# Chris10M/Ev2Hands

Measured on AMD Instinct MI355X. Metric: event-windows/sec at B=256 N=2048 (f16x2), higher is better.
Workload: dtype f32 (each f32 operand split into 2 fp16 planes with per-window power-of-two range scaling, 3 plane products per MAC on the f16 MFMA, f32 accumulate); 1 GPU; TEHNet.forward+MANO both hands, B=256/GPU N=2048 C=4 fp32, E-clouds, random-init 342-key checkpoint, synthetic MANO-shaped assets; global_batch=256, points=2048, channels=4, precision=f16x2, forwards_in_flight=1, world_size_seen=1, parallelism=batch-shard x1

## Files before the change

ev2hands_amd/_lib.py:

```python
from __future__ import annotations

import ctypes as C
import os

_HERE = os.path.dirname(os.path.abspath(__file__))
LIB_PATH = os.environ.get("EV2H_LIB_PATH") or os.path.join(_HERE, "libev2hands_hip.so")

vp = C.c_void_p
ci = C.c_int


class GemmDesc(C.Structure):
    _fields_ = [("X", vp), ("ldx", ci), ("W", vp), ("ldw", ci), ("Y", vp), ("ldy", ci),
                ("M", ci), ("N", ci), ("K", ci),
                ("bias", vp), ("bias_group_rows", ci), ("ldbias", ci), ("relu", ci),
                ("post_scale", vp), ("post_shift", vp),
                ("taps", ci), ("rows_per_seq", ci), ("rowmax_rows", ci), ("precision", ci), ("Ws", vp), ("ws_tile_rows", ci), ("w_unscale", C.c_float),
                ("x_amax", vp), ("x_amax2", vp), ("x_group_rows", ci), ("y_amax", vp), ("y_group_rows", ci), ("y_scale", vp),
                ("y_bound_w", C.c_float), ("y_bound_b", C.c_float), ("skinny", ci)]


class SaDesc(C.Structure):
    _fields_ = [("P1", vp), ("ldp", ci), ("pts4", vp), ("ctr4", vp), ("gidx", vp),
                ("W1x", vp), ("W2", vp), ("b2", vp), ("W3", vp), ("b3", vp),
# ... 45 lines not shown
    _fields_ = [("name", C.c_char_p), ("data", vp), ("dtype", ci), ("ndim", ci), ("shape", C.c_int64 * 4)]


DT_F32, DT_F64, DT_I64 = 0, 1, 2
LOSS_INTER_SHAPE, LOSS_INTER_TRANSL, LOSS_INTER_J3D, LOSS_HAND, LOSS_PER_HAND = 0, 1, 2, 3, 9
LOSS_H_GLOBAL_ORIENT, LOSS_H_HAND_POSE, LOSS_H_SHAPE, LOSS_H_RJ3D, LOSS_H_J3D, LOSS_H_TRANSL, LOSS_H_REG_BETAS, LOSS_H_REG_POSE, LOSS_H_J2D = range(9)
LOSS_NT = LOSS_HAND + 2 * LOSS_PER_HAND
LOSS_NSTATE = LOSS_NT + 6
PACK_EQUALIZE, PACK_HOST_ONLY, PACK_UNEQUALIZED_OK = 1, 2, 4
FAM_SA, FAM_ROWS, FAM_QCONV, FAM_DENSE, FAM_ALL = 1, 2, 4, 8, 15


def pack_f16_families(mask: int) -> int:
    return (int(mask) & 15) << 8
W_EQUALIZED, W_UNEQUALIZED_OK = 1, 2
ABI_VERSION = 8

PREC = {"f32": 0, "bf16": 1, "f16x2": 2, "bf16x3": 3, "f16": 4}


class ManoConsts(C.Structure):
    _fields_ = [("hands_mean", vp), ("comps", vp), ("blend_T", vp), ("v_template", vp),
                ("J_template", vp), ("J_shape", vp), ("weights", vp),
                ("tips", C.c_int32 * 5), ("ncomps", C.c_int32)]


class Outputs(C.Structure):
    _fields_ = [("class_logits", vp), ("params", vp * 2), ("vertices", vp * 2), ("joints", vp * 2),
                ("logits_stride", C.c_size_t), ("params_stride", C.c_size_t), ("vertices_stride", C.c_size_t), ("joints_stride", C.c_size_t)]


EXPORTS = [
    "ev2h_abi_version", "ev2h_source_hash", "ev2h_build_defs", "ev2h_last_error", "ev2h_init", "ev2h_set_side_stream", "ev2h_side_stream_probe", "ev2h_streams_concurrent", "ev2h_bind_stream", "ev2h_shader_clock_probe", "ev2h_struct_sizes",
    "ev2h_prep_points", "ev2h_fps", "ev2h_fps_multi", "ev2h_ball_query", "ev2h_three_nn_interp",
    "ev2h_gemm", "ev2h_transpose_logits", "ev2h_sa_mlp_max", "ev2h_fp_mlp", "ev2h_tile_geometry",
    "ev2h_attn_sim", "ev2h_attn_sim_folded", "ev2h_attn_sim_folded_scratch", "ev2h_attn_context", "ev2h_mano", "ev2h_mano_rotations",
    "ev2h_workspace_bytes", "ev2h_forward", "ev2h_workspace_buffer", "ev2h_workspace_buffer_ex", "ev2h_profile_set", "ev2h_range_report_entries", "ev2h_range_report",
    "ev2h_pack_weights", "ev2h_packed_free", "ev2h_packed_weights", "ev2h_packed_bytes", "ev2h_packed_tensor_count", "ev2h_packed_tensor",
    "ev2h_packed_equalization_count", "ev2h_packed_equalization", "ev2h_packed_weight_spread_count", "ev2h_packed_weight_spread", "ev2h_pack_sa_image_bytes", "ev2h_pack_sa_images",
    "ev2h_pack_gemm_image_bytes", "ev2h_pack_gemm_image", "ev2h_plane_unscale",
    "ev2h_event_window_build", "ev2h_event_window_timesort", "ev2h_event_window_sample", "ev2h_joint_metrics", "ev2h_mesh_collisions", "ev2h_mesh_collisions_ws", "ev2h_mesh_collisions_scratch_bytes", "ev2h_collision_penalty",
    "ev2h_event_window_pixels", "ev2h_demo_point_panels", "ev2h_render_scratch_bytes", "ev2h_render_hands",
    "ev2h_event_stream_links", "ev2h_event_stream_ends", "ev2h_event_stream_walk", "ev2h_event_window_build_ranges",
    "ev2h_event_window_sample_seeded", "ev2h_fps_init_seeded", "ev2h_joint_metrics_frames", "ev2h_eval_accumulate",
    "ev2h_events_undistort",
    "ev2h_event_window_build_s_ranges", "ev2h_joint_metrics_f32_frames", "ev2h_segmentation_score", "ev2h_eval_s_accumulate",
    "ev2h_loss_terms", "ev2h_loss_accumulate",
    "ev2h_event_window_build_s_ranges_aug",
    "ev2h_event_window_build_ranges_flip", "ev2h_finetune_resolve", "ev2h_finetune_targets",
]

_lib = None


class Ev2hError(RuntimeError):
    pass


def lib() -> C.CDLL:
    global _lib
    if _lib is not None:
        return _lib
    import torch
    if not os.path.exists(LIB_PATH):
        raise Ev2hError(f"{LIB_PATH} is missing: build the HIP library first "
                        f"(python -m ev2hands_amd.build). There is no CPU fallback.")
    L = C.CDLL(LIB_PATH)
    if not os.environ.get("EV2H_LIB_PATH"):
        from . import build as _build
        try:
            L.ev2h_source_hash.restype = C.c_char_p
            have = L.ev2h_source_hash().decode()
        except AttributeError:
            have = "(no stamp: built before round 6)"
        want = _build.source_hash()
        if have != want:
            raise Ev2hError(f"{LIB_PATH} was built from other sources (stamp {have[:16]}, sources {want[:16]}): rebuild it "
                            f"(python -m ev2hands_amd.build), or set EV2H_LIB_PATH to use another build on purpose.")
    L.ev2h_last_error.restype = C.c_char_p
    L.ev2h_workspace_bytes.restype = C.c_size_t
    L.ev2h_workspace_bytes.argtypes = [ci, ci]
    L.ev2h_workspace_buffer.restype = vp
    L.ev2h_workspace_buffer.argtypes = [vp, ci, ci, C.c_char_p, C.POINTER(C.c_size_t)]
    L.ev2h_workspace_buffer_ex.restype = vp
    L.ev2h_workspace_buffer_ex.argtypes = [vp, ci, ci, C.c_char_p, C.POINTER(C.c_size_t), C.POINTER(ci)]
    L.ev2h_struct_sizes.restype = None
    L.ev2h_struct_sizes.argtypes = [C.c_size_t * 8]
    L.ev2h_set_side_stream.argtypes = [ci]
    L.ev2h_side_stream_probe.argtypes = [vp, ci, C.POINTER(C.c_float)]
    L.ev2h_shader_clock_probe.argtypes = [vp, ci, vp]
    L.ev2h_streams_concurrent.argtypes = [vp, vp, ci, C.POINTER(C.c_float)]
    L.ev2h_bind_stream.argtypes = [vp, C.POINTER(ci)]
    L.ev2h_prep_points.argtypes = [vp, ci, ci, ci, ci, vp, vp, vp, vp]
    L.ev2h_fps.argtypes = [vp, ci, ci, ci, vp, vp, vp, vp]
    L.ev2h_fps_multi.argtypes = [vp, ci, ci, ci, C.POINTER(ci), C.POINTER(vp), C.POINTER(vp), C.POINTER(vp), vp]
    L.ev2h_ball_query.argtypes = [vp, vp, ci, ci, ci, ci, C.POINTER(C.c_double), C.POINTER(ci), C.POINTER(vp), vp, vp]
    L.ev2h_three_nn_interp.argtypes = [vp, vp, ci, ci, ci, vp, ci, ci, vp, ci, vp, vp, vp, vp]
    L.ev2h_gemm.argtypes = [C.POINTER(GemmDesc), vp]
    L.ev2h_transpose_logits.argtypes = [vp, ci, ci, vp, C.c_size_t, vp]
    L.ev2h_sa_mlp_max.argtypes = [C.POINTER(SaDesc), vp]
    L.ev2h_fp_mlp.argtypes = [C.POINTER(FpDesc), vp]
    L.ev2h_tile_geometry.argtypes = [ci, ci, ci, ci, C.c_int * 10]
    L.ev2h_attn_sim.argtypes = [vp, vp, ci, C.c_size_t, ci, ci, vp, vp]
    L.ev2h_attn_context.argtypes = [vp, vp, ci, ci, ci, vp, vp, ci, vp, vp]
    L.ev2h_attn_sim_folded_scratch.restype = C.c_size_t
    L.ev2h_attn_sim_folded_scratch.argtypes = [ci, ci]
    L.ev2h_attn_sim_folded.argtypes = [vp, vp, ci, ci, ci, vp, vp, vp, vp, vp, vp, vp]
    L.ev2h_mano.argtypes = [C.POINTER(ManoConsts), vp, ci, ci, vp, C.c_size_t, vp, C.c_size_t, vp]
    L.ev2h_mano_rotations.argtypes = [C.POINTER(ManoConsts), vp, ci, ci, vp, vp]
    L.ev2h_forward.argtypes = [C.POINTER(Weights), C.POINTER(ManoConsts), C.POINTER(ManoConsts), vp, ci, ci, ci, ci, vp,
                               C.POINTER(Outputs), vp, C.c_size_t, vp]
    L.ev2h_event_window_build.argtypes = [vp, ci, vp, ci, ci, ci, ci, ci, vp, vp, vp]
    L.ev2h_event_window_timesort.argtypes = [vp, vp, ci, vp, ci, ci, vp, ci, vp, vp, vp]
    L.ev2h_event_window_sample.argtypes = [vp, vp, ci, vp, ci, ci, ci, ci, vp, vp, vp, vp]
    L.ev2h_joint_metrics.argtypes = [vp, vp, vp, ci, ci, ci, C.c_double, vp, vp, vp, vp, vp, vp]
    L.ev2h_mesh_collisions.argtypes = [vp, vp, vp, vp, ci, ci, ci, C.c_float, ci, vp, vp, ci, vp]
    L.ev2h_mesh_collisions_ws.argtypes = [vp, vp, vp, vp, ci, ci, ci, C.c_float, ci, vp, vp, ci, vp, C.c_size_t, vp]
    L.ev2h_mesh_collisions_scratch_bytes.restype = C.c_size_t
    L.ev2h_mesh_collisions_scratch_bytes.argtypes = [ci, ci]
    L.ev2h_collision_penalty.argtypes = [vp, vp, vp, vp, ci, ci, ci, C.c_float, C.c_double, vp, vp, ci, vp, vp]
    L.ev2h_event_stream_links.argtypes = [vp, ci, ci, C.c_double, C.c_double, ci, vp, vp, vp, vp]
    L.ev2h_event_stream_ends.argtypes = [vp, ci, ci, vp, vp, ci, ci, vp, vp]
    L.ev2h_event_stream_walk.argtypes = [vp, vp, ci, ci, vp, ci, vp, vp, vp, vp]
    L.ev2h_events_undistort.argtypes = [vp, ci, ci, C.POINTER(C.c_double), C.POINTER(C.c_double), ci, ci, ci, vp, vp]
    L.ev2h_event_window_build_ranges.argtypes = [vp, ci, ci, vp, vp, ci, ci, ci, ci, ci, vp, vp, vp, vp, vp]
    L.ev2h_event_window_build_ranges_flip.argtypes = [vp, ci, ci, vp, vp, ci, ci, ci, ci, ci, C.c_uint64, vp, vp, vp, vp, vp, vp, vp]
    L.ev2h_finetune_resolve.argtypes = [vp, ci, ci, vp, vp, ci, vp, vp, ci, C.c_uint64, ci, ci, ci] + [vp] * 9 + [vp]
    L.ev2h_finetune_targets.argtypes = [vp, ci, vp, vp, ci, vp, vp, vp, vp, vp, vp, ci, vp, ci, ci] + [vp] * 8 + [vp]
    L.ev2h_event_window_sample_seeded.argtypes = [vp, vp, ci, C.c_uint64, vp, ci, ci, ci, ci, vp, vp, vp, vp, vp, vp]
    L.ev2h_fps_init_seeded.argtypes = [C.c_uint64, vp, ci, ci, ci, vp, vp]
# ... 133 lines not shown
```

ev2hands_amd/csrc/forward.hip:

```cpp
#include <cstdarg>
#include <cstdio>
#include <cstdlib>
#include <cstring>

#include "common.hpp"
#include "planes.hpp"
#include "ev2hands_hip.h"
#include "side_stream.hpp"
#include "workspace.hpp"

int ev2h_gemm_init();

static thread_local char g_err[512] = "";

void ev2h_set_error(const char* fmt, ...) {
    va_list ap;
    va_start(ap, fmt);
    vsnprintf(g_err, sizeof(g_err), fmt, ap);
    va_end(ap);
}

extern "C" const char* ev2h_last_error(void) { return g_err; }
extern "C" int ev2h_abi_version(void) { return EV2H_ABI_VERSION; }

// ... 150 lines not shown
        extra = fmaxf(extra, m.br[i].w1x_norm * (float)m.br[i].radius * 1.0000002f);
    }
    ev2h_gemm_desc g{};
    g.X = feat; g.ldx = ldf; g.W = m.W1f; g.ldw = m.kf; g.Y = P1; g.ldy = c1sum;
    g.M = B * Npts; g.N = c1sum; g.K = m.kf; g.bias = m.b1; g.taps = 1;
    g.precision = precision;
    g.w_unscale = m.w1f_unscale;
    if (precision != EV2H_PREC_F32 && m.W1fs) { g.Ws = m.W1fs; g.ws_tile_rows = 128; }
    if (feat_amax) {
        g.x_amax = feat_amax; g.x_group_rows = Npts;
        g.y_amax = p1_amax; g.y_group_rows = Npts;
        g.y_scale = p1_scale; g.y_bound_w = m.w1f_norm; g.y_bound_b = m.b1_max + extra;
        if (precision == EV2H_PREC_F16 && chain) {
            float wmul = 1.f, badd = g.y_bound_b;
            for (int i = 0; i < m.nbranch; ++i) {
                const float iu = 1.000001f / (m.br[i].w2_unscale > 0.f ? m.br[i].w2_unscale : 1.f);
                wmul = fmaxf(wmul, m.br[i].w2_norm * iu);
                badd = fmaxf(badd, (m.br[i].w2_norm * g.y_bound_b + m.br[i].b2_max) * iu);
            }
            g.y_bound_w *= wmul; g.y_bound_b = badd;
        }
    }
    return ev2h_gemm(&g, st);
}

static bool bf16_direct_layer1(int precision, const ev2h_sa_module& m) {
    static const bool table = getenv("EV2H_L1_TABLE") != nullptr;
    return precision != EV2H_PREC_F32 && m.kf == 8 && !table;
}

static int sa_branches(int precision, const char* tag, const ev2h_sa_module& m, const float* pts4, const float* ctr4, int32_t* const* gidx,
                       const int32_t* cnt, int B, int Npts, const float* P1, float* out, int ldo, ev2h_stream_t st, bool ranges,
                       const uint32_t* p1_amax, const float* p1_scale, uint32_t* out_amax, const float* feat = nullptr, int nfeat = 0,
                       const uint32_t* feat_amax = nullptr, float* xyz_out = nullptr, int xyz_ld = 0, int s_off = 0, int s_cnt = 0) {
    int c1sum = 0;
    for (int i = 0; i < m.nbranch; ++i) c1sum += m.br[i].C1;
    int coff1 = 0, coff3 = 0;
    for (int i = 0; i < m.nbranch; ++i) {
        const ev2h_sa_branch& br = m.br[i];
        ev2h_sa_desc d{};
        d.P1 = P1 + coff1; d.ldp = c1sum; d.pts4 = pts4; d.ctr4 = ctr4; d.gidx = gidx[i];
        d.W1x = br.W1x; d.W2 = br.W2; d.b2 = br.b2; d.W3 = br.W3; d.b3 = br.b3;
        d.out = out + coff3; d.ldo = ldo;
        d.B = B; d.Npts = Npts; d.S = m.npoint; d.K = br.K; d.C1 = br.C1; d.C2 = br.C2; d.C3 = br.C3;
        if (s_cnt > 0) { d.S = s_cnt; d.S_total = m.npoint; d.s_off = s_off; }
        d.precision = precision; d.W2s = br.W2s; d.W3s = br.W3s; d.w2_unscale = br.w2_unscale; d.w3_unscale = br.w3_unscale;
        const bool direct = feat && bf16_direct_layer1(precision, m);
        if (direct) {
            d.feat = feat; d.ldf = 8; d.W1f = m.W1f + (size_t)coff1 * m.kf; d.ldw1f = m.kf; d.b1 = m.b1 + coff1; d.nfeat = nfeat;
            d.w1f_unscale = br.w1f_unscale; d.w1x_unscale = br.w1x_unscale;
            if (ranges) { d.feat_amax = feat_amax; d.w1f_norm = m.w1f_norm; d.b1_max = m.b1_max; }
        }
        if (ranges) {
            if (!direct) { d.p1_scale = p1_scale; d.p1_amax = p1_amax; }
            d.out_amax = out_amax;
            d.w1x_norm = br.w1x_norm; d.dmax = (float)br.radius * 1.0000002f ; d.w2_norm = br.w2_norm; d.b2_max = br.b2_max;
        }
        d.cnt = cnt ? cnt + i : nullptr; d.cnt_ld = m.nbranch;
        if (i == 0 && xyz_out) { d.xyz_out = xyz_out; d.xyz_ld = xyz_ld; }
        char t[40];
        snprintf(t, sizeof(t), "%s.%d", tag, i);
        prof_begin(t, st);
        RUN(ev2h_sa_mlp_max(&d, st));
        prof_end(t, st);
        coff1 += br.C1;
        coff3 += br.C3;
    }
    return EV2H_OK;
}

static int sa_module(int precision, const char* tag, const ev2h_sa_module& m, const float* feat, int ldf, const float* pts4, const float* ctr4,
                     int32_t* const* gidx, const int32_t* cnt, int B, int Npts, float* P1, float* out, int ldo, ev2h_stream_t st,
                     const uint32_t* feat_amax, uint32_t* p1_amax, float* p1_scale, uint32_t* out_amax, int nfeat = 0, float* xyz_out = nullptr,
                     int xyz_ld = 0) {
    if (!bf16_direct_layer1(precision, m)) RUN(sa_table(precision, m, feat, ldf, B, Npts, P1, st, feat_amax, p1_amax, p1_scale));
    return sa_branches(precision, tag, m, pts4, ctr4, gidx, cnt, B, Npts, P1, out, ldo, st, feat_amax != nullptr, p1_amax, p1_scale, out_amax,
                       ldf == 8 ? feat : nullptr, nfeat, feat_amax, xyz_out, xyz_ld);
}

}

static int forward_body(const ev2h_weights* w, const ev2h_mano_consts* const* mano, float* xyz_cm, int B, int C, int N, int mhlnes,
                        const int64_t* fps_init, const ev2h_outputs* out, const Call& cx, bool* forked) {
    const Ws& ws = cx.ws;
    const ev2h_stream_t st = cx.st;
    const int R = B * N;
    const int prec = cx.prec;
    const int prec_sa = cx.fam_prec(EV2H_FAM_SA), prec_rows = cx.fam_prec(EV2H_FAM_ROWS), prec_q = cx.fam_prec(EV2H_FAM_QCONV);
    auto rg = [&](int xid, int xg, int yid = -1, int yg = 0, int xid2 = -1) {
        Rng r{};
        if (ws.ranges_on) {
            r.xa = ws.r(xid); r.xg = xg;
            if (xid2 >= 0) r.xa2 = ws.r(xid2);
            if (yid >= 0) { r.ya = ws.r(yid); r.yg = yg; }
        }
        return r;
    };
    if (ws.ranges_on) EV2H_CHECK_HIP(hipMemsetAsync(ws.i(WS_RANGES), 0, ws.L.count[WS_RANGES] * 4, (hipStream_t)st));

    RUN(ev2h_prep_points(xyz_cm, B, C, N, mhlnes, ws.f(WS_PTS4), ws.f(WS_FEAT8), ws.r(R_FEAT), st));
    const bool fork = cx.side != nullptr;
    const ev2h_stream_t sd = fork ? (ev2h_stream_t)cx.side->stream : st;
    RUN(cx.signal_side(EV_INPUT));
    *forked = fork;
    if (!bf16_direct_layer1(prec, w->sa1)) RUN(sa_table(prec_sa, w->sa1, ws.f(WS_FEAT8), 8, B, N, ws.f(WS_P1A), sd, ws.r(R_FEAT), ws.r(R_P1A), ws.p1scale(0)));
    RUN(cx.side_records(EV_SA1_TABLE));
    static const int chunk_env = [] { const char* e = getenv("EV2H_FPS_CHUNKS"); return e ? atoi(e) : -1; }();
    const int chunk_max_wg = chunk_env > 1 ? chunk_env : (N <= 2048 ? 0x7fffffff : 256), chunk_min_b = chunk_env > 1 ? 1 : 8;
    const bool chunked = fork && chunk_env != 0 && B >= chunk_min_b && 3 * B <= chunk_max_wg && bf16_direct_layer1(prec, w->sa1) && w->sa1.npoint % FPS_CHUNKS == 0;
    const bool side_queries = chunked && B >= 64 && N <= 2048;
    int32_t* gi1[3] = {ws.i(WS_GIDX1_0), ws.i(WS_GIDX1_1), ws.i(WS_GIDX1_2)};
    double rad1[3]; int ns1[3];
    for (int i = 0; i < 3; ++i) { rad1[i] = w->sa1.br[i].radius; ns1[i] = w->sa1.br[i].K; }
    const int S[3] = {512, 128, 128};
    const int64_t* init[3] = {fps_init, fps_init + 2 * (size_t)B, fps_init + 3 * (size_t)B};
    int32_t* idx[3] = {ws.i(WS_FPS1), ws.i(WS_FPSM_L), ws.i(WS_FPSM_R)};
    float* ctr[3] = {ws.f(WS_CTR1), ws.f(WS_CTRM_L), ws.f(WS_CTRM_R)};
    static const bool unfused_fp1 = getenv("EV2H_FP1_UNFUSED") != nullptr;
    const bool fp1_fused = prec != EV2H_PREC_F32 && w->fp1m.W1fs && !unfused_fp1;
    auto late_selections = [&](bool with_samplings) -> int {
        if (fp1_fused) {
            RUN(ev2h_three_nn_interp(ws.f(WS_PTS4), ws.f(WS_CTR1), B, N, 512, nullptr, 0, 0, nullptr, 0, ws.i(WS_NN1_IDX), ws.f(WS_NN1_W), nullptr, sd));
            RUN(cx.side_records(EV_FP1_NN));
        }
        if (with_samplings) RUN(ev2h_fps_multi(ws.f(WS_PTS4), B, N, 2, S + 1, init + 1, idx + 1, ctr + 1, sd));
        for (int h = 0; h < 2; ++h) {
            const ev2h_sa_module& m = w->mano_sa1[h];
            double rad[2]; int ns[2];
            int32_t* gi[2] = {ws.i(hand(WS_GIDXM0_L, h)), ws.i(hand(WS_GIDXM1_L, h))};
            for (int i = 0; i < 2; ++i) { rad[i] = m.br[i].radius; ns[i] = m.br[i].K; }
            RUN(ev2h_ball_query(ws.f(WS_PTS4), ws.f(hand(WS_CTRM_L, h)), B, N, 128, 2, rad, ns, gi, ws.i(hand(WS_CNTM_L, h)), sd));
        }
        return cx.side_records(EV_HAND_QUERIES);
    };
    if (!chunked) {
        RUN(ev2h_fps_multi(ws.f(WS_PTS4), B, N, 3, S, init, idx, ctr, st));
    } else {
        const int q = w->sa1.npoint / FPS_CHUNKS;
        for (int c = 0; c < FPS_CHUNKS; ++c) {
            RUN(ev2h_fps_multi_chunk(ws.f(WS_PTS4), B, N, side_queries ? 1 : 3, S, init, idx, ctr, c * q, (c + 1) * q, ws.f(WS_FPS_STATE), sd));
            if (side_queries) RUN(ev2h_ball_query_range(ws.f(WS_PTS4), ws.f(WS_CTR1), B, N, 512, c * q, q, 3, rad1, ns1, gi1, ws.i(WS_CNT1), sd));
            RUN(cx.side_records(EV_SA1_QUARTER0 + c));
        }
    }
    if (!chunked) RUN(cx.signal_side(EV_SAMPLED));
    int32_t* gi2[2] = {ws.i(WS_GIDX2_0), ws.i(WS_GIDX2_1)};
    {
        const ev2h_sa_module& m = w->sa2;
        RUN(ev2h_fps(ws.f(WS_CTR1), B, 512, 128, fps_init + (size_t)B, ws.i(WS_FPS2), ws.f(WS_CTR2), sd));
        double rad[2]; int ns[2];
        for (int i = 0; i < 2; ++i) { rad[i] = m.br[i].radius; ns[i] = m.br[i].K; }
        RUN(ev2h_ball_query(ws.f(WS_CTR1), ws.f(WS_CTR2), B, 512, 128, 2, rad, ns, gi2, ws.i(WS_CNT2), sd));
        RUN(cx.side_records(EV_SA2_QUERY));
    }
    if (!side_queries) RUN(late_selections(false));
    {
        const ev2h_sa_module& m = w->sa1;
        if (!chunked) {
            RUN(ev2h_ball_query(ws.f(WS_PTS4), ws.f(WS_CTR1), B, N, 512, 3, rad1, ns1, gi1, ws.i(WS_CNT1), st));
            RUN(cx.wait_side(EV_SA1_TABLE));
            RUN(sa_branches(prec_sa, "sa1", m, ws.f(WS_PTS4), ws.f(WS_CTR1), gi1, ws.i(WS_CNT1), B, N, ws.f(WS_P1A), ws.f(WS_L1CAT), 576, st, ws.ranges_on,
                            ws.r(R_P1A), ws.p1scale(0), ws.r(R_L1A), ws.f(WS_FEAT8), C, ws.r(R_FEAT)));
        } else {
            const int q = m.npoint / FPS_CHUNKS;
            for (int c = 0; c < FPS_CHUNKS; ++c) {
                RUN(cx.wait_side(EV_SA1_QUARTER0 + c));
                if (!side_queries) RUN(ev2h_ball_query_range(ws.f(WS_PTS4), ws.f(WS_CTR1), B, N, 512, c * q, q, 3, rad1, ns1, gi1, ws.i(WS_CNT1), st));
                RUN(sa_branches(prec_sa, "sa1", m, ws.f(WS_PTS4), ws.f(WS_CTR1), gi1, ws.i(WS_CNT1), B, N, ws.f(WS_P1A), ws.f(WS_L1CAT), 576, st, ws.ranges_on,
                                ws.r(R_P1A), ws.p1scale(0), ws.r(R_L1A), ws.f(WS_FEAT8), C, ws.r(R_FEAT), nullptr, 0, c * q, q));
            }
        }
    }
    {
        const ev2h_sa_module& m = w->sa2;
        RUN(cx.wait_side(EV_SA2_QUERY));
        RUN(sa_module(prec_sa, "sa2", m, ws.f(WS_L1CAT), 576, ws.f(WS_CTR1), ws.f(WS_CTR2), gi2, ws.i(WS_CNT2), B, 512, ws.f(WS_P1B), ws.f(WS_L2BUF), 520, st,
                      ws.r(R_L1A), ws.r(R_P1B), ws.p1scale(1), ws.r(R_L2), 0, ws.f(WS_L2BUF) + 512, 520));
    }
    RUN(dense(cx, w->sa3[0], ws.f(WS_L2BUF), 520, B * 128, ws.f(WS_SA3H1), 256, 1, st, rg(R_L2, 128, R_SA3H1, 128, R_FEAT)));
    RUN(dense(cx, w->sa3[1], ws.f(WS_SA3H1), 256, B * 128, ws.f(WS_SA3H2), 512, 1, st, rg(R_SA3H1, 128, R_SA3H2, 128)));
    RUN(dense(cx, w->sa3[2], ws.f(WS_SA3H2), 512, B * 128, ws.f(WS_L3), 1024, 1, st, rg(R_SA3H2, 128, R_L3, 1), {.rowmax_rows = 128}));
    RUN(dense(cx, w->fp3_bcast, ws.f(WS_L3), 1024, B, ws.f(WS_FP3BIAS), 256, 0, st, rg(R_L3, 1), {.skinny = 1}));
    if (side_queries) {
        RUN(cx.signal_side(EV_ENC_SA3));
        RUN(late_selections(true));
    }
    RUN(dense(cx, w->fp3_skip, ws.f(WS_L2BUF), 520, B * 128, ws.f(WS_FP3H), 256, 1, st, rg(R_L2, 128, R_FP3H, 128, R_FEAT),
              {.group_bias = ws.f(WS_FP3BIAS), .group_rows = 128, .ldbias = 256}));
    RUN(dense(cx, w->fp3_1, ws.f(WS_FP3H), 256, B * 128, ws.f(WS_FP3O), 256, 1, st, rg(R_FP3H, 128, R_FP3O, 128)));
    RUN(ev2h_three_nn_interp(ws.f(WS_CTR1), ws.f(WS_CTR2), B, 512, 128, ws.f(WS_FP3O), 256, 256, ws.f(WS_L1CAT) + 320, 576,
                             ws.i(WS_NN2_IDX), ws.f(WS_NN2_W), ws.r(R_L1B), st));
    RUN(dense(cx, w->fp2[0], ws.f(WS_L1CAT), 576, B * 512, ws.f(WS_FP2H), 256, 1, st, rg(R_L1A, 512, R_FP2H, 512, R_L1B)));
    RUN(dense(cx, w->fp2[1], ws.f(WS_FP2H), 256, B * 512, ws.f(WS_L1NEW), 128, 1, st, rg(R_FP2H, 512, R_L1NEW, 512)));
    static const bool unfused_cls = getenv("EV2H_CLS_UNFUSED") != nullptr;
    static const bool unfused_zsum = getenv("EV2H_ATTN_UNFUSED_ZSUM") != nullptr;
    static const bool l0_f32 = getenv("EV2H_L0_F32") != nullptr;
    const bool cls_fused = prec != EV2H_PREC_F32 && w->clsm.W2s && !unfused_cls;
    const ev2h_gemm_desc qd = dense_desc(cx, w->qconv0, ws.f(WS_L0), 256, R, ws.f(WS_Q1), 512, 1, rg(R_L0, N),
                                         {.taps = 3, .rows_per_seq = N, .fam = EV2H_FAM_QCONV});
    const bool zsum_ok = !unfused_zsum && prec != EV2H_PREC_F32 && w->qconv0.Ws && ev2h_gemm_bf16_zsum_supported(&qd);
    const bool l0_bf16 = prec == EV2H_PREC_BF16 && fp1_fused && cls_fused && zsum_ok && !l0_f32;
    const bool l0_f16 = prec == EV2H_PREC_F16 && prec_rows == EV2H_PREC_F16 && prec_q == EV2H_PREC_F16 && ws.ranges_on && fp1_fused && cls_fused && zsum_ok && !l0_f32;
    const bool l0_16 = l0_bf16 || l0_f16;
    g_last_l0_bf16 = l0_bf16 ? 1 : (l0_f16 ? 2 : 0);
    if (fp1_fused) {
        const ev2h_sa_module& m = w->fp1m;
        RUN(cx.wait_side(EV_FP1_NN));
        RUN(sa_table(prec_rows, m, ws.f(WS_L1NEW), 128, B, 512, ws.f(WS_FP1T), st, ws.r(R_L1NEW), ws.r(R_FP1T), ws.p1scale(4), false));
        ev2h_fp_desc d{};
        d.T = ws.f(WS_FP1T); d.ldt = 128; d.nn_idx = ws.i(WS_NN1_IDX); d.nn_w = ws.f(WS_NN1_W);
        d.b2 = m.br[0].b2; d.b3 = m.br[0].b3; d.W2s = m.br[0].W2s; d.W3s = m.br[0].W3s;
        d.w2_unscale = m.br[0].w2_unscale; d.w3_unscale = m.br[0].w3_unscale;
        d.out = ws.f(WS_L0); d.ldo = 256; d.B = B; d.N = N; d.S = 512; d.C1 = 128; d.C2 = 128; d.C3 = 256; d.precision = prec_rows;
        if (ws.ranges_on) {
            d.t_scale = ws.p1scale(4); d.t_amax = ws.r(R_FP1T); d.w2_norm = m.br[0].w2_norm; d.b2_max = m.br[0].b2_max; d.out_amax = ws.r(R_L0);
        }
        prof_begin("fp1", st);
        RUN(ev2h_fp_mlp_ex(&d, 0, l0_16, st, l0_f16 ? ws.p1scale(5) : nullptr, m.br[0].w3_norm, m.br[0].b3_max));
        prof_end("fp1", st);
    } else {
        RUN(ev2h_three_nn_interp(ws.f(WS_PTS4), ws.f(WS_CTR1), B, N, 512, ws.f(WS_L1NEW), 128, 128, ws.f(WS_FP1IN), 128,
                                 ws.i(WS_NN1_IDX), ws.f(WS_NN1_W), ws.r(R_FP1IN), st));
        RUN(dense(cx, w->fp1[0], ws.f(WS_FP1IN), 128, R, ws.f(WS_FP1H1), 128, 1, st, rg(R_FP1IN, N, R_FP1H1, N)));
        RUN(dense(cx, w->fp1[1], ws.f(WS_FP1H1), 128, R, ws.f(WS_FP1H2), 128, 1, st, rg(R_FP1H1, N, R_FP1H2, N)));
// ... 115 lines not shown
```

ev2hands_amd/csrc/points.hip:

```cpp
#include <cstdlib>
#include "common.hpp"
#include "ev2hands_hip.h"

namespace {

typedef float f32x2 __attribute__((ext_vector_type(2)));

__device__ __forceinline__ float sqnorm3(float x, float y, float z) {
    return __fadd_rn(__fadd_rn(__fmul_rn(x, x), __fmul_rn(y, y)), __fmul_rn(z, z));
}

__global__ __launch_bounds__(256) void prep_points_kernel(float* __restrict__ xyz_cm, int C, int N, int mhlnes,
                                                          float4* __restrict__ pts4, float4* __restrict__ feat8,
                                                          unsigned* __restrict__ amax) {
    const int b = blockIdx.y;
    const int n = blockIdx.x * 256 + threadIdx.x;
    float* base = xyz_cm + (size_t)b * C * N;
    float f[8];
#pragma unroll
    for (int c = 0; c < 8; ++c) f[c] = (c < C && n < N) ? base[(size_t)c * N + n] : 0.f;
    if (mhlnes && n < N) {
        float s = f[3];
        for (int c = 4; c < C; ++c) s = __fadd_rn(s, f[c]);
        s = s / (float)(C - 3);
// ... 264 lines not shown
        for (int c = lane; c < D4; c += 64) {
            float4 a[4], bq[4], cq[4];
            float w0[4], w1[4], w2[4];
#pragma unroll
            for (int u = 0; u < 4; ++u) {
                const int t = t0 + u;
                const int j0 = sidx[t * 3 + 0], j1 = sidx[t * 3 + 1], j2 = sidx[t * 3 + 2];
                w0[u] = sw[t * 3 + 0]; w1[u] = sw[t * 3 + 1]; w2[u] = sw[t * 3 + 2];
                const bool live = blockIdx.x * ppw + t < N1;
                a[u] = reinterpret_cast<const float4*>(feat2 + ((size_t)b * N2 + (live ? j0 : 0)) * ldf2)[c];
                bq[u] = reinterpret_cast<const float4*>(feat2 + ((size_t)b * N2 + (live ? j1 : 0)) * ldf2)[c];
                cq[u] = reinterpret_cast<const float4*>(feat2 + ((size_t)b * N2 + (live ? j2 : 0)) * ldf2)[c];
            }
#pragma unroll
            for (int u = 0; u < 4; ++u) {
                const int nn = blockIdx.x * ppw + t0 + u;
                if (nn >= N1) break;
                float4 r;
                r.x = __fadd_rn(__fadd_rn(__fmul_rn(a[u].x, w0[u]), __fmul_rn(bq[u].x, w1[u])), __fmul_rn(cq[u].x, w2[u]));
                r.y = __fadd_rn(__fadd_rn(__fmul_rn(a[u].y, w0[u]), __fmul_rn(bq[u].y, w1[u])), __fmul_rn(cq[u].y, w2[u]));
                r.z = __fadd_rn(__fadd_rn(__fmul_rn(a[u].z, w0[u]), __fmul_rn(bq[u].z, w1[u])), __fmul_rn(cq[u].z, w2[u]));
                r.w = __fadd_rn(__fadd_rn(__fmul_rn(a[u].w, w0[u]), __fmul_rn(bq[u].w, w1[u])), __fmul_rn(cq[u].w, w2[u]));
                reinterpret_cast<float4*>(out + ((size_t)b * N1 + nn) * ldo)[c] = r;
                am = fmaxf(fmaxf(am, fmaxf(fabsf(r.x), fabsf(r.y))), fmaxf(fabsf(r.z), fabsf(r.w)));
            }
        }
    }
    if (amax) {
        const unsigned m = wave_max_u32_dpp(__float_as_uint(am));
        if (lane == 0 && m) atomicMax(&amax[b], m);
    }
}

}

extern "C" int ev2h_prep_points(float* xyz_cm, int B, int C, int N, int mhlnes, float* pts4, float* feat8, uint32_t* amax,
                                ev2h_stream_t stream) {
    EV2H_CHECK_ARG(xyz_cm && pts4 && feat8);
    EV2H_CHECK_ARG(B > 0 && N > 0 && C >= 4 && C <= 8);
    dim3 grid(ceil_div(N, 256), B);
    prep_points_kernel<<<grid, 256, 0, (hipStream_t)stream>>>(xyz_cm, C, N, mhlnes, (float4*)pts4, (float4*)feat8, amax);
    EV2H_CHECK_LAUNCH();
    return EV2H_OK;
}

size_t ev2h_fps_state_ld(int N) {
    const int threads = N <= 2048 ? 256 : (N <= 8192 ? 512 : 1024);
    const int ppt = N <= 256 ? 1 : N <= 512 ? 2 : N <= 1024 ? 4 : N <= 2048 ? 8 : N <= 4096 ? 8 : N <= 8192 ? 16 : N <= 16384 ? 16 : 32;
    return (size_t)threads * ppt + 4;
}

int ev2h_fps_multi_chunk(const float* pts4, int B, int N, int njobs, const int* S, const int64_t* const* init, int32_t* const* idx, float* const* ctr4,
                         int s_begin, int s_end, float* state, ev2h_stream_t stream);

extern "C" int ev2h_fps_multi(const float* pts4, int B, int N, int njobs, const int* S, const int64_t* const* init,
                              int32_t* const* idx, float* const* ctr4, ev2h_stream_t stream) {
    return ev2h_fps_multi_chunk(pts4, B, N, njobs, S, init, idx, ctr4, 0, 0x7fffffff, nullptr, stream);
}

int ev2h_fps_multi_chunk(const float* pts4, int B, int N, int njobs, const int* S, const int64_t* const* init, int32_t* const* idx, float* const* ctr4,
                         int s_begin, int s_end, float* state, ev2h_stream_t stream) {
    EV2H_CHECK_ARG(pts4 && S && init && idx && ctr4);
    EV2H_CHECK_ARG(B > 0 && N > 0 && N <= 32768 && njobs >= 1 && njobs <= 3);
    EV2H_CHECK_ARG(s_begin >= 0 && s_end > s_begin);
    FpsJobs jobs{};
    jobs.njobs = njobs;
// ... 54 lines not shown
        a.r2[i] = (float)(radius[i] * radius[i]);
        a.K[i] = nsample[i];
        a.gidx[i] = gidx[i];
    }
    a.cnt = cnt;
    a.cpw = BALL_CTR_PER_WG;
    a.s_off = s_off; a.s_cnt = s_cnt;
    a.nchunk = ceil_div(s_cnt, a.cpw);
    ball_query_kernel<<<dim3((unsigned)a.nchunk * (unsigned)B), 256, 0, (hipStream_t)stream>>>((const float4*)pts4, (const float4*)ctr4, N, S, a);
    EV2H_CHECK_LAUNCH();
    return EV2H_OK;
}

extern "C" int ev2h_three_nn_interp(const float* pts1_4, const float* pts2_4, int B, int N1, int N2, const float* feat2,
                                    int ldf2, int D, float* out, int ldo, int32_t* nn_idx, float* nn_w, uint32_t* out_amax,
                                    ev2h_stream_t stream) {
    EV2H_CHECK_ARG(pts1_4 && pts2_4);
    EV2H_CHECK_ARG(B > 0 && N1 > 0 && N2 >= 3 && N2 <= NN_MAX_N2);
    if (out) EV2H_CHECK_ARG(feat2 && D > 0 && (D % 4) == 0 && (ldf2 % 4) == 0 && (ldo % 4) == 0);
    const int ppw = ((long)ceil_div(N1, NN_PTS_PER_WG) * B < 128) ? 64 : NN_PTS_PER_WG;
    dim3 grid(ceil_div(N1, ppw), B);
    const size_t lds = (size_t)N2 * sizeof(float4) + NN_PTS_PER_WG * 3 * (sizeof(int) + sizeof(float));
    if (lds > 64 * 1024) {
        static PerDevice attr_set{};
        EV2H_ONCE_PER_DEVICE(attr_set,
            EV2H_CHECK_HIP(hipFuncSetAttribute(reinterpret_cast<const void*>(three_nn_interp_kernel), hipFuncAttributeMaxDynamicSharedMemorySize,
                                               NN_MAX_N2 * (int)sizeof(float4) + NN_PTS_PER_WG * 3 * (int)(sizeof(int) + sizeof(float)))););
    }
    three_nn_interp_kernel<<<grid, 256, lds, (hipStream_t)stream>>>((const float4*)pts1_4, (const float4*)pts2_4, N1, N2, feat2,
                                                                    ldf2, D, out, ldo, nn_idx, nn_w, out_amax, ppw);
    EV2H_CHECK_LAUNCH();
    return EV2H_OK;
}
```

ev2hands_amd/csrc/side_stream.hpp:

```cpp
#pragma once
#include "common.hpp"
#include "ev2hands_hip.h"

constexpr int FPS_CHUNKS = 4;

enum SideEvent {
    EV_SAMPLED,
    EV_HAND_QUERIES,
    EV_HF8,
    EV_JOIN,
    EV_INPUT,
    EV_SA1_TABLE,
    EV_L0,
    EV_LOGITS,
    EV_SA2_QUERY,
    EV_FP1_NN,
    EV_ENC_SA3,
    EV_SA1_QUARTER0,
    EV_COUNT = 15
};
static_assert(EV_SA1_QUARTER0 + FPS_CHUNKS == EV_COUNT, "one event per chunk of enc.sa1's sampling");

struct SideCtx {
    hipStream_t stream = nullptr;
    hipEvent_t ev[EV_COUNT] = {};
    int state = 0;
    void* owner = nullptr;
    bool claimed = false;
    bool bound = false;
    unsigned long long last_use = 0;
};

SideCtx* ev2h_side_ctx(void* caller_stream, bool claim);
extern thread_local int g_side_disabled;
```

include/ev2hands_hip.h:

```cpp
#ifndef EV2HANDS_HIP_H
#define EV2HANDS_HIP_H

#include <stddef.h>
#include <stdint.h>

#ifdef __cplusplus
extern "C" {
#endif

#define EV2H_ABI_VERSION 8

typedef void* ev2h_stream_t;

#define EV2H_PREC_F32 0
#define EV2H_PREC_BF16 1
#define EV2H_PREC_F16X2 2
#define EV2H_PREC_BF16X3 3
#define EV2H_PREC_F16 4


int ev2h_abi_version(void);
const char* ev2h_source_hash(void);
const char* ev2h_build_defs(void);
const char* ev2h_last_error(void);
int ev2h_init(void);
int ev2h_set_side_stream(int enabled);
int ev2h_side_stream_probe(ev2h_stream_t stream, int spin_us, float* ratio);
int ev2h_streams_concurrent(ev2h_stream_t a, ev2h_stream_t b, int spin_us, float* ratio);
int ev2h_bind_stream(ev2h_stream_t stream, int* info);
int ev2h_shader_clock_probe(ev2h_stream_t stream, int spin_us, unsigned long long* out_dev);
void ev2h_struct_sizes(size_t out[8]);

int ev2h_prep_points(float* xyz_cm, int B, int C, int N, int mhlnes, float* pts4, float* feat8, uint32_t* feat_amax,
                     ev2h_stream_t stream);

int ev2h_fps(const float* pts4, int B, int N, int S, const int64_t* init, int32_t* idx, float* ctr4, ev2h_stream_t stream);
int ev2h_fps_multi(const float* pts4, int B, int N, int njobs, const int* S, const int64_t* const* init,
                   int32_t* const* idx, float* const* ctr4, ev2h_stream_t stream);

int ev2h_ball_query(const float* pts4, const float* ctr4, int B, int N, int S, int nrad, const double* radius,
                    const int* nsample, int32_t* const* gidx, int32_t* cnt, ev2h_stream_t stream);

int ev2h_three_nn_interp(const float* pts1_4, const float* pts2_4, int B, int N1, int N2, const float* feat2, int ldf2,
                         int D, float* out, int ldo, int32_t* nn_idx, float* nn_w, uint32_t* out_amax, ev2h_stream_t stream);

typedef struct ev2h_gemm_desc {
    const float* X; int ldx;
    const float* W; int ldw;
    float* Y; int ldy;
    int M, N, K;
    const float* bias;
    int bias_group_rows;
    int ldbias;
    int relu;
    const float* post_scale;
    const float* post_shift;
    int taps;
    int rows_per_seq;
    int rowmax_rows;
    int precision;
    const void* Ws;
    int ws_tile_rows;
    float w_unscale;
    const uint32_t* x_amax;
    const uint32_t* x_amax2;
    int x_group_rows;
    uint32_t* y_amax;
    int y_group_rows;
    float* y_scale;
    float y_bound_w, y_bound_b;
    int skinny;
} ev2h_gemm_desc;
int ev2h_gemm(const ev2h_gemm_desc* d, ev2h_stream_t stream);

int ev2h_transpose_logits(const float* logits_pm, int B, int N, float* logits_cm, size_t cm_window_stride, ev2h_stream_t stream);

typedef struct ev2h_sa_desc {
// ... 324 lines not shown
```

Before: 23260 event-windows/s.

## Overlap SA1 narrow branch and FP2 neighbour search on the side stream

Moves the first (narrow) SA1 branch MLP onto the side stream per FPS chunk when the batch is large, so the main stream runs only the remaining branches and then waits on a new event. It also splits FP2's three-NN interpolation: the neighbour search runs on the side stream right after the SA2 ball query, and the main stream later applies a new blend-only kernel using the precomputed indices and weights. The aim is to hide the SA1 branch and the NN search behind main-stream work, at the cost of more events, extra cross-stream sync and contention for compute units.

```diff
diff --git a/ev2hands_amd/_lib.py b/ev2hands_amd/_lib.py
--- a/ev2hands_amd/_lib.py
+++ b/ev2hands_amd/_lib.py
@@ -101,7 +101,7 @@
 
 EXPORTS = [
     "ev2h_abi_version", "ev2h_source_hash", "ev2h_build_defs", "ev2h_last_error", "ev2h_init", "ev2h_set_side_stream", "ev2h_side_stream_probe", "ev2h_streams_concurrent", "ev2h_bind_stream", "ev2h_shader_clock_probe", "ev2h_struct_sizes",
-    "ev2h_prep_points", "ev2h_fps", "ev2h_fps_multi", "ev2h_ball_query", "ev2h_three_nn_interp",
+    "ev2h_prep_points", "ev2h_fps", "ev2h_fps_multi", "ev2h_ball_query", "ev2h_three_nn_interp", "ev2h_three_nn_blend",
     "ev2h_gemm", "ev2h_transpose_logits", "ev2h_sa_mlp_max", "ev2h_fp_mlp", "ev2h_tile_geometry",
     "ev2h_attn_sim", "ev2h_attn_sim_folded", "ev2h_attn_sim_folded_scratch", "ev2h_attn_context", "ev2h_mano", "ev2h_mano_rotations",
     "ev2h_workspace_bytes", "ev2h_forward", "ev2h_workspace_buffer", "ev2h_workspace_buffer_ex", "ev2h_profile_set", "ev2h_range_report_entries", "ev2h_range_report",
@@ -165,6 +165,7 @@
     L.ev2h_fps_multi.argtypes = [vp, ci, ci, ci, C.POINTER(ci), C.POINTER(vp), C.POINTER(vp), C.POINTER(vp), vp]
     L.ev2h_ball_query.argtypes = [vp, vp, ci, ci, ci, ci, C.POINTER(C.c_double), C.POINTER(ci), C.POINTER(vp), vp, vp]
     L.ev2h_three_nn_interp.argtypes = [vp, vp, ci, ci, ci, vp, ci, ci, vp, ci, vp, vp, vp, vp]
+    L.ev2h_three_nn_blend.argtypes = [vp, vp, ci, ci, ci, vp, ci, ci, vp, ci, vp, vp]
     L.ev2h_gemm.argtypes = [C.POINTER(GemmDesc), vp]
     L.ev2h_transpose_logits.argtypes = [vp, ci, ci, vp, C.c_size_t, vp]
     L.ev2h_sa_mlp_max.argtypes = [C.POINTER(SaDesc), vp]
diff --git a/ev2hands_amd/csrc/forward.hip b/ev2hands_amd/csrc/forward.hip
--- a/ev2hands_amd/csrc/forward.hip
+++ b/ev2hands_amd/csrc/forward.hip
@@ -206,11 +206,14 @@
 static int sa_branches(int precision, const char* tag, const ev2h_sa_module& m, const float* pts4, const float* ctr4, int32_t* const* gidx,
                        const int32_t* cnt, int B, int Npts, const float* P1, float* out, int ldo, ev2h_stream_t st, bool ranges,
                        const uint32_t* p1_amax, const float* p1_scale, uint32_t* out_amax, const float* feat = nullptr, int nfeat = 0,
-                       const uint32_t* feat_amax = nullptr, float* xyz_out = nullptr, int xyz_ld = 0, int s_off = 0, int s_cnt = 0) {
+                       const uint32_t* feat_amax = nullptr, float* xyz_out = nullptr, int xyz_ld = 0, int s_off = 0, int s_cnt = 0,
+                       int br_first = 0, int br_end = -1) {
+    if (br_end < 0) br_end = m.nbranch;
     int c1sum = 0;
     for (int i = 0; i < m.nbranch; ++i) c1sum += m.br[i].C1;
     int coff1 = 0, coff3 = 0;
-    for (int i = 0; i < m.nbranch; ++i) {
+    for (int i = 0; i < m.nbranch; coff1 += m.br[i].C1, coff3 += m.br[i].C3, ++i) {
+        if (i < br_first || i >= br_end) continue;
         const ev2h_sa_branch& br = m.br[i];
         ev2h_sa_desc d{};
         d.P1 = P1 + coff1; d.ldp = c1sum; d.pts4 = pts4; d.ctr4 = ctr4; d.gidx = gidx[i];
@@ -237,8 +240,6 @@
         prof_begin(t, st);
         RUN(ev2h_sa_mlp_max(&d, st));
         prof_end(t, st);
-        coff1 += br.C1;
-        coff3 += br.C3;
     }
     return EV2H_OK;
 }
@@ -283,6 +284,8 @@
     const int chunk_max_wg = chunk_env > 1 ? chunk_env : (N <= 2048 ? 0x7fffffff : 256), chunk_min_b = chunk_env > 1 ? 1 : 8;
     const bool chunked = fork && chunk_env != 0 && B >= chunk_min_b && 3 * B <= chunk_max_wg && bf16_direct_layer1(prec, w->sa1) && w->sa1.npoint % FPS_CHUNKS == 0;
     const bool side_queries = chunked && B >= 64 && N <= 2048;
+    const bool narrow_side = side_queries && B >= 128;
+    const bool fp2_split = fork && B >= 16;
     int32_t* gi1[3] = {ws.i(WS_GIDX1_0), ws.i(WS_GIDX1_1), ws.i(WS_GIDX1_2)};
     double rad1[3]; int ns1[3];
     for (int i = 0; i < 3; ++i) { rad1[i] = w->sa1.br[i].radius; ns1[i] = w->sa1.br[i].K; }
@@ -315,7 +318,11 @@
             RUN(ev2h_fps_multi_chunk(ws.f(WS_PTS4), B, N, side_queries ? 1 : 3, S, init, idx, ctr, c * q, (c + 1) * q, ws.f(WS_FPS_STATE), sd));
             if (side_queries) RUN(ev2h_ball_query_range(ws.f(WS_PTS4), ws.f(WS_CTR1), B, N, 512, c * q, q, 3, rad1, ns1, gi1, ws.i(WS_CNT1), sd));
             RUN(cx.side_records(EV_SA1_QUARTER0 + c));
-        }
+            if (narrow_side)
+                RUN(sa_branches(prec_sa, "sa1", w->sa1, ws.f(WS_PTS4), ws.f(WS_CTR1), gi1, ws.i(WS_CNT1), B, N, ws.f(WS_P1A), ws.f(WS_L1CAT), 576, sd, ws.ranges_on,
+                                ws.r(R_P1A), ws.p1scale(0), ws.r(R_L1A), ws.f(WS_FEAT8), C, ws.r(R_FEAT), nullptr, 0, c * q, q, 0, 1));
+        }
+        if (narrow_side) RUN(cx.side_records(EV_SA1_NARROW));
     }
     if (!chunked) RUN(cx.signal_side(EV_SAMPLED));
     int32_t* gi2[2] = {ws.i(WS_GIDX2_0), ws.i(WS_GIDX2_1)};
@@ -326,6 +333,10 @@
         for (int i = 0; i < 2; ++i) { rad[i] = m.br[i].radius; ns[i] = m.br[i].K; }
         RUN(ev2h_ball_query(ws.f(WS_CTR1), ws.f(WS_CTR2), B, 512, 128, 2, rad, ns, gi2, ws.i(WS_CNT2), sd));
         RUN(cx.side_records(EV_SA2_QUERY));
+        if (fp2_split) {
+            RUN(ev2h_three_nn_interp(ws.f(WS_CTR1), ws.f(WS_CTR2), B, 512, 128, nullptr, 0, 0, nullptr, 0, ws.i(WS_NN2_IDX), ws.f(WS_NN2_W), nullptr, sd));
+            RUN(cx.side_records(EV_FP2_NN));
+        }
     }
     if (!side_queries) RUN(late_selections(false));
     {
@@ -341,8 +352,9 @@
                 RUN(cx.wait_side(EV_SA1_QUARTER0 + c));
                 if (!side_queries) RUN(ev2h_ball_query_range(ws.f(WS_PTS4), ws.f(WS_CTR1), B, N, 512, c * q, q, 3, rad1, ns1, gi1, ws.i(WS_CNT1), st));
                 RUN(sa_branches(prec_sa, "sa1", m, ws.f(WS_PTS4), ws.f(WS_CTR1), gi1, ws.i(WS_CNT1), B, N, ws.f(WS_P1A), ws.f(WS_L1CAT), 576, st, ws.ranges_on,
-                                ws.r(R_P1A), ws.p1scale(0), ws.r(R_L1A), ws.f(WS_FEAT8), C, ws.r(R_FEAT), nullptr, 0, c * q, q));
+                                ws.r(R_P1A), ws.p1scale(0), ws.r(R_L1A), ws.f(WS_FEAT8), C, ws.r(R_FEAT), nullptr, 0, c * q, q, narrow_side ? 1 : 0));
             }
+            if (narrow_side) RUN(cx.wait_side(EV_SA1_NARROW));
         }
     }
     {
@@ -362,8 +374,13 @@
     RUN(dense(cx, w->fp3_skip, ws.f(WS_L2BUF), 520, B * 128, ws.f(WS_FP3H), 256, 1, st, rg(R_L2, 128, R_FP3H, 128, R_FEAT),
               {.group_bias = ws.f(WS_FP3BIAS), .group_rows = 128, .ldbias = 256}));
     RUN(dense(cx, w->fp3_1, ws.f(WS_FP3H), 256, B * 128, ws.f(WS_FP3O), 256, 1, st, rg(R_FP3H, 128, R_FP3O, 128)));
-    RUN(ev2h_three_nn_interp(ws.f(WS_CTR1), ws.f(WS_CTR2), B, 512, 128, ws.f(WS_FP3O), 256, 256, ws.f(WS_L1CAT) + 320, 576,
-                             ws.i(WS_NN2_IDX), ws.f(WS_NN2_W), ws.r(R_L1B), st));
+    if (fp2_split) {
+        RUN(cx.wait_side(EV_FP2_NN));
+        RUN(ev2h_three_nn_blend(ws.i(WS_NN2_IDX), ws.f(WS_NN2_W), B, 512, 128, ws.f(WS_FP3O), 256, 256, ws.f(WS_L1CAT) + 320, 576, ws.r(R_L1B), st));
+    } else {
+        RUN(ev2h_three_nn_interp(ws.f(WS_CTR1), ws.f(WS_CTR2), B, 512, 128, ws.f(WS_FP3O), 256, 256, ws.f(WS_L1CAT) + 320, 576,
+                                 ws.i(WS_NN2_IDX), ws.f(WS_NN2_W), ws.r(R_L1B), st));
+    }
     RUN(dense(cx, w->fp2[0], ws.f(WS_L1CAT), 576, B * 512, ws.f(WS_FP2H), 256, 1, st, rg(R_L1A, 512, R_FP2H, 512, R_L1B)));
     RUN(dense(cx, w->fp2[1], ws.f(WS_FP2H), 256, B * 512, ws.f(WS_L1NEW), 128, 1, st, rg(R_FP2H, 512, R_L1NEW, 512)));
     static const bool unfused_cls = getenv("EV2H_CLS_UNFUSED") != nullptr;
diff --git a/ev2hands_amd/csrc/points.hip b/ev2hands_amd/csrc/points.hip
--- a/ev2hands_amd/csrc/points.hip
+++ b/ev2hands_amd/csrc/points.hip
@@ -320,6 +320,62 @@
     }
 }
 
+constexpr int NN_BLEND_PTS = 64;
+template <int PTS>
+__global__ __launch_bounds__(256) void three_nn_blend_kernel(const int32_t* __restrict__ nn_idx, const float* __restrict__ nn_w, int N1, int N2,
+                                                             const float* __restrict__ feat2, int ldf2, int D, float* __restrict__ out, int ldo,
+                                                             unsigned* __restrict__ amax, int nchunk) {
+    static_assert(PTS % 16 == 0, "four waves, four points per iteration");
+    const int L = xcd_remap(blockIdx.x, gridDim.x);
+    const int b = L / nchunk, chunk = L - b * nchunk;
+    const int lane = threadIdx.x & 63, wave = __builtin_amdgcn_readfirstlane(threadIdx.x >> 6);
+    const int D4 = D >> 2;
+    constexpr int pw = PTS / 4;
+    float am = 0.f;
+#pragma unroll 1
+    for (int t0 = wave * pw; t0 < wave * pw + pw; t0 += 4) {
+        const int n0 = chunk * PTS + t0;
+        if (n0 >= N1) break;
+        int j[4][3];
+        float w[4][3];
+#pragma unroll
+        for (int u = 0; u < 4; ++u) {
+            const size_t r = ((size_t)b * N1 + min(n0 + u, N1 - 1)) * 3;
+#pragma unroll
+            for (int k = 0; k < 3; ++k) { j[u][k] = (int)min((unsigned)nn_idx[r + k], (unsigned)(N2 - 1)); w[u][k] = nn_w[r + k]; }
+        }
+        auto four = [&](auto tail) {
+            constexpr bool TAIL = decltype(tail)::value;
+            for (int c = lane; c < D4; c += 64) {
+                float4 a[4], bq[4], cq[4];
+#pragma unroll
+                for (int u = 0; u < 4; ++u) {
+                    a[u] = reinterpret_cast<const float4*>(feat2 + ((size_t)b * N2 + j[u][0]) * ldf2)[c];
+                    bq[u] = reinterpret_cast<const float4*>(feat2 + ((size_t)b * N2 + j[u][1]) * ldf2)[c];
+                    cq[u] = reinterpret_cast<const float4*>(feat2 + ((size_t)b * N2 + j[u][2]) * ldf2)[c];
+                }
+#pragma unroll
+                for (int u = 0; u < 4; ++u) {
+                    if (TAIL && n0 + u >= N1) break;
+                    float4 r;
+                    r.x = __fadd_rn(__fadd_rn(__fmul_rn(a[u].x, w[u][0]), __fmul_rn(bq[u].x, w[u][1])), __fmul_rn(cq[u].x, w[u][2]));
+                    r.y = __fadd_rn(__fadd_rn(__fmul_rn(a[u].y, w[u][0]), __fmul_rn(bq[u].y, w[u][1])), __fmul_rn(cq[u].y, w[u][2]));
+                    r.z = __fadd_rn(__fadd_rn(__fmul_rn(a[u].z, w[u][0]), __fmul_rn(bq[u].z, w[u][1])), __fmul_rn(cq[u].z, w[u][2]));
+                    r.w = __fadd_rn(__fadd_rn(__fmul_rn(a[u].w, w[u][0]), __fmul_rn(bq[u].w, w[u][1])), __fmul_rn(cq[u].w, w[u][2]));
+                    reinterpret_cast<float4*>(out + ((size_t)b * N1 + n0 + u) * ldo)[c] = r;
+                    am = fmaxf(fmaxf(am, fmaxf(fabsf(r.x), fabsf(r.y))), fmaxf(fabsf(r.z), fabsf(r.w)));
+                }
+            }
+        };
+        if (n0 + 4 <= N1) four(std::false_type{});
+        else four(std::true_type{});
+    }
+    if (amax) {
+        const unsigned m = wave_max_u32_dpp(__float_as_uint(am));
+        if (lane == 0 && m) atomicMax(&amax[b], m);
+    }
+}
+
 }
 
 extern "C" int ev2h_prep_points(float* xyz_cm, int B, int C, int N, int mhlnes, float* pts4, float* feat8, uint32_t* amax,
@@ -440,3 +496,15 @@
     EV2H_CHECK_LAUNCH();
     return EV2H_OK;
 }
+
+extern "C" int ev2h_three_nn_blend(const int32_t* nn_idx, const float* nn_w, int B, int N1, int N2, const float* feat2, int ldf2, int D,
+                                   float* out, int ldo, uint32_t* out_amax, ev2h_stream_t stream) {
+    EV2H_CHECK_ARG(nn_idx && nn_w && feat2 && out);
+    EV2H_CHECK_ARG(B > 0 && N1 > 0 && N2 >= 3 && D > 0 && (D % 4) == 0 && (ldf2 % 4) == 0 && (ldo % 4) == 0 && ldf2 >= D && ldo >= D);
+    const int nchunk = ceil_div(N1, NN_BLEND_PTS);
+    EV2H_CHECK_ARG((long)nchunk * B <= 0x7fffffffL);
+    three_nn_blend_kernel<NN_BLEND_PTS><<<dim3((unsigned)nchunk * (unsigned)B), 256, 0, (hipStream_t)stream>>>(nn_idx, nn_w, N1, N2, feat2, ldf2, D, out, ldo,
+                                                                                                             out_amax, nchunk);
+    EV2H_CHECK_LAUNCH();
+    return EV2H_OK;
+}
diff --git a/ev2hands_amd/csrc/side_stream.hpp b/ev2hands_amd/csrc/side_stream.hpp
--- a/ev2hands_amd/csrc/side_stream.hpp
+++ b/ev2hands_amd/csrc/side_stream.hpp
@@ -15,11 +15,13 @@
     EV_LOGITS,
     EV_SA2_QUERY,
     EV_FP1_NN,
+    EV_FP2_NN,
     EV_ENC_SA3,
     EV_SA1_QUARTER0,
-    EV_COUNT = 15
+    EV_SA1_NARROW = EV_SA1_QUARTER0 + FPS_CHUNKS,
+    EV_COUNT = 17
 };
-static_assert(EV_SA1_QUARTER0 + FPS_CHUNKS == EV_COUNT, "one event per chunk of enc.sa1's sampling");
+static_assert(EV_SA1_NARROW + 1 == EV_COUNT, "one event per chunk of enc.sa1's sampling, then the narrow branch's");
 
 struct SideCtx {
     hipStream_t stream = nullptr;
diff --git a/include/ev2hands_hip.h b/include/ev2hands_hip.h
--- a/include/ev2hands_hip.h
+++ b/include/ev2hands_hip.h
@@ -43,6 +43,9 @@
 
 int ev2h_three_nn_interp(const float* pts1_4, const float* pts2_4, int B, int N1, int N2, const float* feat2, int ldf2,
                          int D, float* out, int ldo, int32_t* nn_idx, float* nn_w, uint32_t* out_amax, ev2h_stream_t stream);
+
+int ev2h_three_nn_blend(const int32_t* nn_idx, const float* nn_w, int B, int N1, int N2, const float* feat2, int ldf2, int D,
+                        float* out, int ldo, uint32_t* out_amax, ev2h_stream_t stream);
 
 typedef struct ev2h_gemm_desc {
     const float* X; int ldx;
```

Result: no change. 23400 event-windows/s (median of 6 runs) (+0.6%).
